# jasonppy/VoiceCraft

Hardware: NVIDIA H100
Metric: codec tokens/s (830M TTS decode) (higher is better)
Workload: dtype bf16

## Files before the change

voicecraft_b200/csrc/lm_engine.cu:

```cuda
#include "../../include/vcb200.h"
#include "lm_kernels.cuh"

#include <algorithm>
#include <array>
#include <cstdarg>
#include <cstdio>
#include <cstdlib>
#include <cstring>
#include <map>
#include <utility>

namespace vcb {

static thread_local char g_err[1024] = "";
void set_error(const char* fmt, ...) {
    va_list ap;
    va_start(ap, fmt);
    vsnprintf(g_err, sizeof(g_err), fmt, ap);
    va_end(ap);
}
const char* get_error() { return g_err; }

__global__ void f32_to_bf16_kernel(const float* __restrict__ in, __nv_bfloat16* __restrict__ out, size_t n) {
    for (size_t i = blockIdx.x * static_cast<size_t>(blockDim.x) + threadIdx.x; i < n;
// ... 106 lines not shown
    DevBuf<__nv_bfloat16> mact_d, mact_d2, mact_f, mact_h;
    DevBuf<int> mega_att_cnt;
    int64_t n_launches = 0;
    struct ProfRec { int cls; Event a, b; };
    std::vector<ProfRec> prof;
    std::vector<Event> ev_pool;
    Event get_event() {
        Event ev;
        if (ev_pool.empty()) {
            ev.create();
        } else {
            ev = std::move(ev_pool.back());
            ev_pool.pop_back();
        }
        return ev;
    }

    ~vcb_engine() {
        cudaSetDevice(cfg.device);
        cudaDeviceSynchronize();
    }
};

enum { PC_GEMM = 0, PC_ATTN = 1, PC_LN = 2, PC_FINISH = 3, PC_SAMPLER = 4, PC_MISC = 5, PC_MEGA = 6, PC_N = 7 };

struct ProfScope {
    vcb_engine* e; cudaStream_t st; int idx = -1;
    ProfScope(vcb_engine* e_, int cls, cudaStream_t st_) : e(e_), st(st_) {
        if (!e->opt_profile) return;
        vcb_engine::ProfRec r{cls, e->get_event(), e->get_event()};
        cudaEventRecord(r.a, st);
        e->prof.push_back(std::move(r));
        idx = static_cast<int>(e->prof.size()) - 1;
    }
    ~ProfScope() { if (idx >= 0) cudaEventRecord(e->prof[idx].b, st); }
};

namespace {

int bpad_for(int rows) { return rows <= 16 ? 16 : rows <= 32 ? 32 : rows <= 64 ? 64 : 128; }
int bpad_idx(int bpad) { return bpad == 16 ? 0 : bpad == 32 ? 1 : bpad == 64 ? 2 : 3; }

int pack_matrix(const float* src, Matrix* M, int rows, int cols) {
    if (M->w.ensure(packed_weight_elems(rows, cols))) return -1;
    M->rows = rows;
    M->cols = cols;
    return pack_weight(src, M->w, rows, cols, &M->tm);
}

int to_bf16_matrix(vcb_engine* e, const std::string& key, Matrix* M, int rows, int cols) {
    auto it = e->f32.find(key);
    if (it == e->f32.end()) {
        set_error("missing weight %s", key.c_str());
        return -1;
    }
    const auto& sh = e->shapes[key];
    if (sh.size() != 2 || sh[0] != rows || sh[1] != cols) {
        set_error("weight %s has wrong shape", key.c_str());
        return -1;
    }
    return pack_matrix(it->second, M, rows, cols);
}

int need(vcb_engine* e, const std::string& key, float** out, size_t numel) {
    auto it = e->f32.find(key);
    if (it == e->f32.end()) {
        set_error("missing weight %s", key.c_str());
        return -1;
    }
    size_t n = 1;
    for (auto s : e->shapes[key]) n *= static_cast<size_t>(s);
    if (n != numel) {
        set_error("weight %s: expected %zu elements, got %zu", key.c_str(), numel, n);
        return -1;
    }
    *out = it->second;
    return 0;
}

int upload_ints(vcb_engine* e, const int* src, size_t n, int* dst, cudaStream_t st) {
    if (n > e->h_stage_ints) {
        set_error("staging overflow");
        return -1;
    }
    VCB_CUDA_OK(cudaEventSynchronize(e->stage_ev));
    memcpy(e->h_stage, src, n * sizeof(int));
    VCB_CUDA_OK(cudaMemcpyAsync(dst, e->h_stage, n * sizeof(int), cudaMemcpyHostToDevice, st));
    VCB_CUDA_OK(cudaEventRecord(e->stage_ev, st));
    return 0;
}

#define LAUNCH_COUNT(e) ((e)->n_launches++)

template <typename... KArgs, typename... Args>
cudaError_t launch_k(vcb_engine* e, void (*kern)(KArgs...), dim3 grid, dim3 block, size_t smem, cudaStream_t st,
                     Args&&... args) {
    return launch_k_pdl(e->opt_pdl, kern, grid, block, smem, st, std::forward<Args>(args)...);
}

int decode_splits(int s, int Nout, int bpad, int maxctas) {
    if (bpad >= 64 && s > 1) s /= 2;
    if (maxctas > 0) {
        const int tiles = (Nout + 127) / 128;
        while (s > 1 && tiles * s > maxctas) s /= 2;
    }
    while (s > 1 && bpad % s) s /= 2;
    return s;
}

int run_gemm(vcb_engine* e, const Matrix& W, const CUtensorMap* tmB, const __nv_bfloat16* X, int ldx, int bpad,
             int nvalid, int b_col_off, int kdim, const GemmEpilogue& ep, cudaStream_t st, const Matrix* next = nullptr) {
    GemmCall g;
    if (next && e->opt_prefetch) {
        g.pf_ptr = next->w;
        g.pf_bytes = packed_weight_elems(next->rows, next->cols) * 2;
        if (e->opt_prefetch == 2) g.pf_bytes |= (1ull << 63);
    }
    g.tmA = &W.tm;
    g.tmB = tmB;
    g.W = W.w;
    g.X = X;
    g.ep = ep;
    g.Nout = W.rows;
    g.Kdim = kdim;
    g.ldx = ldx;
    g.bpad = bpad;
    int splits = gemm_pick_splits(W.rows, kdim, e->num_sms);
    for (const auto& o : e->opt_splits)
        if (o[0] == W.rows && o[1] == kdim) splits = o[2];
    g.splits = decode_splits(splits, W.rows, bpad, e->opt_gemm_maxctas);
    g.stages = e->opt_gemm_stages;
    g.b_col_off = b_col_off;
    g.nvalid = nvalid;
    g.pdl = e->opt_pdl;
    g.simt = e->opt_simt;
    LAUNCH_COUNT(e);
    ProfScope ps(e, PC_GEMM, st);
    return gemm_launch(g, st);
}

struct AttnLaunch {
    const float* q = nullptr;
    const void *kpool = nullptr, *vpool = nullptr;
    const int *page_table = nullptr, *row_slot = nullptr, *row_pos = nullptr;
    const int* row_pages = nullptr;
    int max_pages = 0, rows = 0, H = 0, hd = 0, kv_fp32 = 0, max_ctx = 0;
    __nv_bfloat16* act = nullptr;
    int ld_act = 0, bpad = 0;
    float* ws = nullptr;
    int* cnt = nullptr;
    int maxch = 1, chunk_pages = 16, num_sms = 132, balance = 1, pdl = 0;
    const int *grp_first = nullptr, *grp_shared = nullptr;
    int n_groups = 0;
};

template <typename KVT, int HD, int GMAX>
int launch_attn_hd(const AttnLaunch& a, cudaStream_t st) {
    const float scale = 1.0f / sqrtf(static_cast<float>(HD));
    using L = AttSmem<KVT, HD>;
    static bool set = false;
    if (!set) {
        VCB_CUDA_OK(cudaFuncSetAttribute(attn_rows_kernel<KVT, HD, GMAX>, cudaFuncAttributeMaxDynamicSharedMemorySize, L::TOTAL));
        set = true;
    }
    const int npages = (a.max_ctx + KV_PAGE - 1) / KV_PAGE;
    const int nch = std::min(a.maxch, std::max(1, (npages + a.chunk_pages - 1) / a.chunk_pages));
    const int n_rh = (GMAX == 1 ? a.rows : a.n_groups) * a.H;
    const int per_sm = std::max(1, std::min(4, (227 * 1024) / (L::TOTAL + 1024)));
    int grid = std::min(n_rh * nch, a.num_sms * per_sm);
    if (a.balance) {
        const int items = n_rh * nch, passes = (items + grid - 1) / grid;
        grid = (items + passes - 1) / passes;
    }
    VCB_CUDA_OK(launch_k_pdl(a.pdl, attn_rows_kernel<KVT, HD, GMAX>, dim3(grid), dim3(ATT_THREADS + 32), L::TOTAL, st, a.q,
                             static_cast<const KVT*>(a.kpool), static_cast<const KVT*>(a.vpool), a.page_table, a.max_pages,
                             a.row_slot, a.row_pos, a.H, a.act, a.ld_act, a.bpad, scale, a.ws, a.cnt, a.maxch, a.chunk_pages,
                             n_rh, nch, a.row_pages, a.grp_first, a.grp_shared));
    return 0;
}

template <typename KVT, int HD>
int launch_attn_kv(const AttnLaunch& a, cudaStream_t st) {
    return a.n_groups > 0 ? launch_attn_hd<KVT, HD, ATT_GMAX>(a, st) : launch_attn_hd<KVT, HD, 1>(a, st);
}

int launch_attn_rows(const AttnLaunch& a, cudaStream_t st) {
    if (a.hd != 64 && a.hd != 128) {
        set_error("attention: head dim %d (64 or 128 supported)", a.hd);
        return -1;
    }
    if (a.kv_fp32)
        return a.hd == 128 ? launch_attn_kv<float, 128>(a, st) : launch_attn_kv<float, 64>(a, st);
    return a.hd == 128 ? launch_attn_kv<__nv_bfloat16, 128>(a, st) : launch_attn_kv<__nv_bfloat16, 64>(a, st);
}

struct Plane {
    __nv_bfloat16* act = nullptr;
    const CUtensorMap* tm = nullptr;
};

struct Pass {
    int rows = 0;
    int bpad = 0;
    int max_ctx = 1;
    bool fold = false;
    bool wide = false;
    const int *slot = nullptr, *pos = nullptr, *last = nullptr, *page = nullptr;
    const int* pages = nullptr;
    const int* forced = nullptr;
    const int *grp_first = nullptr, *grp_shared = nullptr;
    int n_groups = 0;
    float* x = nullptr;
    const int* x_index = nullptr;
    float* q = nullptr;
    Plane act_d, act_d2, act_f, act_h;
    float* att_ws = nullptr;
    int* att_cnt = nullptr;
};

Pass narrow_pass(vcb_engine* e, int rows, bool fold) {
    Pass p;
    p.rows = rows;
    p.bpad = bpad_for(rows);
    const int bi = bpad_idx(p.bpad);
    p.fold = fold;
    p.x = e->x_rows;
    p.q = e->qbuf;
    p.act_d = {e->act_d, &e->tm_act_d[bi]};
    p.act_d2 = {e->act_d2, &e->tm_act_d2[bi]};
    p.act_f = {e->act_f, &e->tm_act_f[bi]};
    p.act_h = {e->act_h, &e->tm_act_h[bi]};
    p.att_ws = e->att_ws;
    p.att_cnt = e->att_cnt;
    return p;
}

Pass step_pass(vcb_engine* e, int n, bool fold) {
    Pass p = narrow_pass(e, n, fold);
    p.slot = e->row_slot;
    p.pos = e->row_pos;
    p.last = e->row_last;
    p.page = e->row_page;
    p.pages = e->row_pages;
    p.forced = e->row_forced;
    p.n_groups = e->n_row_groups;
    p.grp_first = e->d_slots + n;
    p.grp_shared = p.grp_first + p.n_groups + 1;
    return p;
}

Pass wide_pass(vcb_engine* e, int rows) {
    Pass p;
    p.rows = rows;
    p.bpad = e->wide_rows;
    p.wide = true;
    p.x = e->wx;
    p.q = e->wq;
    p.act_d = {e->wact_d, &e->tm_wact_d};
    p.act_f = {e->wact_f, &e->tm_wact_f};
    p.att_ws = e->w_att_ws;
    p.att_cnt = e->w_att_cnt;
    return p;
}

void fold_epilogue(GemmEpilogue& ep, const float* cvec, const float* bprime, const float* stats, int tiles, int d) {
    ep.ln_fold = 1;
    ep.cvec = cvec;
    ep.bias = bprime;
    ep.stats = stats;
    ep.stats_tiles = tiles;
    ep.inv_d = 1.0f / static_cast<float>(d);
    ep.ln_d = d;
    ep.ln_eps = 1e-5f;
}

void emit_epilogue(GemmEpilogue& ep, const float* gamma_next, __nv_bfloat16* dst, int d, int bpad, float* stats) {
    ep.emit = 1;
    ep.next_gamma = gamma_next;
    ep.next_act = dst;
    ep.next_ld = d;
    ep.next_bpad = bpad;
    ep.stats_out = stats;
}

struct LayerEpilogues {
    GemmEpilogue qkv, out, ff1, ff2;
};

LayerEpilogues layer_epilogues(const vcb_engine* e, int l, const Pass& p) {
    const ModelDims& m = e->m;
    const Layer& Ly = e->layers[l];
    const int dtiles = (m.d + 127) / 128;
    LayerEpilogues r;
    GemmEpilogue& q = r.qkv;
    q.mode = EPI_QKV;
    q.bias = Ly.b_qkv;
    q.qbuf = p.q;
    q.kpool = Ly.kpool;
    q.vpool = Ly.vpool;
    q.page_table = e->page_table;
    q.row_slot = p.slot;
    q.row_pos = p.pos;
    q.row_page = p.page;
    q.kv_fp32 = e->kv_fp32;
    q.max_pages = e->max_pages_per_slot;
    q.page_size = KV_PAGE;
    q.d = m.d;
    q.H = m.H;
    q.hd = m.hd;
    r.out.mode = EPI_RESID;
    r.out.bias = Ly.b_out;
    r.out.x = p.x;
    r.out.ld_out = m.d;
    r.ff1.mode = EPI_ACT;
    r.ff1.bias = Ly.b_ff1;
    r.ff1.act = p.act_f.act;
    r.ff1.ld_out = m.F;
    r.ff1.act_kind = 1;
    r.ff1.bpad_out = p.bpad;
    r.ff2.mode = EPI_RESID;
    r.ff2.bias = Ly.b_ff2;
    r.ff2.x = p.x;
    r.ff2.ld_out = m.d;
    if (p.fold) {
        fold_epilogue(r.qkv, Ly.c_qkv, Ly.bp_qkv, e->ln_stats, l == 0 ? 1 : dtiles, m.d);
        emit_epilogue(r.out, Ly.ln2_g, p.act_d2.act, m.d, p.bpad, e->ln_stats);
        fold_epilogue(r.ff1, Ly.c_ff1, Ly.bp_ff1, e->ln_stats, dtiles, m.d);
        emit_epilogue(r.ff2, l + 1 < m.L ? e->layers[l + 1].ln1_g : e->lnf_g, p.act_d.act, m.d, p.bpad, e->ln_stats);
    }
    return r;
}

GemmEpilogue heads_epilogue(const vcb_engine* e, const Pass& p) {
    const ModelDims& m = e->m;
    GemmEpilogue ep;
    ep.mode = EPI_ACT;
    ep.bias = e->b_h1;
    ep.act = p.act_h.act;
    ep.ld_out = m.K * m.Hh;
    ep.act_kind = 2;
    ep.bpad_out = p.bpad;
    if (p.fold) fold_epilogue(ep, e->c_h1, e->bp_h1, e->ln_stats, (m.d + 127) / 128, m.d);
    return ep;
}

int pass_gemm(vcb_engine* e, const Pass& p, const Matrix& W, const Plane& in, const GemmEpilogue& ep, cudaStream_t st,
              const Matrix* next) {
    if (!p.wide) return run_gemm(e, W, in.tm, in.act, W.cols, p.bpad, p.rows, 0, W.cols, ep, st, next);
    RowsGemmCall g;
    g.tmX = in.tm;
    g.tmW = &W.tm;
    g.ep = ep;
    g.rows = p.rows;
    g.rcap = p.bpad;
    g.Nout = W.rows;
    g.Kdim = W.cols;
    g.pdl = e->opt_pdl;
    LAUNCH_COUNT(e);
    ProfScope ps(e, PC_GEMM, st);
    return gemm_rows_launch(g, st);
}

int launch_attn(vcb_engine* e, const Pass& p, const Layer& Ly, cudaStream_t st) {
    const ModelDims& m = e->m;
    AttnLaunch a;
    a.q = p.q;
    a.kpool = Ly.kpool;
    a.vpool = Ly.vpool;
    a.page_table = e->page_table;
    a.row_slot = p.slot;
    a.row_pos = p.pos;
    a.row_pages = p.pages;
    a.max_pages = e->max_pages_per_slot;
    a.rows = p.rows;
    a.H = m.H;
    a.hd = m.hd;
    a.kv_fp32 = e->kv_fp32;
    a.max_ctx = p.max_ctx;
    a.act = p.act_d.act;
    a.ld_act = m.d;
    a.bpad = p.bpad;
    a.ws = p.att_ws;
    a.cnt = p.att_cnt;
    a.maxch = e->att_maxch;
    a.chunk_pages = e->att_chunk_pages;
    a.num_sms = e->num_sms;
    a.balance = e->opt_att_balance;
    a.pdl = e->opt_pdl;
    a.grp_first = p.grp_first;
    a.grp_shared = p.grp_shared;
    a.n_groups = p.n_groups;
    ProfScope ps(e, PC_ATTN, st);
    if (launch_attn_rows(a, st)) return -1;
    LAUNCH_COUNT(e);
    return 0;
}

int launch_ln(vcb_engine* e, const Pass& p, const float* g, const float* b, cudaStream_t st) {
    const int d = e->m.d;
    ProfScope ps(e, PC_LN, st);
    auto* kern = d <= 2048 ? ln_rows_kernel<8> : ln_rows_kernel<16>;
    VCB_CUDA_OK(launch_k(e, kern, dim3(p.rows), dim3(256), 0, st, p.x, p.x_index, g, b, p.act_d.act, d, p.bpad, d, 1e-5f));
    LAUNCH_COUNT(e);
    return 0;
}

int forward_layers(vcb_engine* e, const Pass& p, cudaStream_t st) {
    const ModelDims& m = e->m;
    for (int l = 0; l < m.L; ++l) {
        const Layer& Ly = e->layers[l];
        const LayerEpilogues ep = layer_epilogues(e, l, p);
        if (!p.fold && launch_ln(e, p, Ly.ln1_g, Ly.ln1_b, st)) return -1;
        if (pass_gemm(e, p, Ly.qkv, p.act_d, ep.qkv, st, &Ly.out) || launch_attn(e, p, Ly, st) ||
            pass_gemm(e, p, Ly.out, p.act_d, ep.out, st, &Ly.ff1))
            return -1;
        if (!p.fold && launch_ln(e, p, Ly.ln2_g, Ly.ln2_b, st)) return -1;
        if (pass_gemm(e, p, Ly.ff1, p.fold ? p.act_d2 : p.act_d, ep.ff1, st, &Ly.ff2) ||
            pass_gemm(e, p, Ly.ff2, p.act_f, ep.ff2, st, l + 1 < m.L ? &e->layers[l + 1].qkv : &e->h1))
            return -1;
    }
    return 0;
}

bool wide_usable(const vcb_engine* e) {
    const ModelDims& m = e->m;
    return e->opt_prefill_wide && !e->opt_simt && m.hd % 32 == 0 && gemm_rows_supported(3 * m.d, m.d, m.hd) &&
           gemm_rows_supported(m.F, m.d, 0) && gemm_rows_supported(m.d, m.F, 0) && (m.hd == 128 || m.hd == 64);
}

int wide_alloc(vcb_engine* e) {
    const ModelDims& m = e->m;
    const size_t W = static_cast<size_t>(e->wide_rows);
    auto grab = [](auto& buf, size_t n) {
        if (!buf.ensure(n, true)) return false;
        set_error("wide prefill: out of device memory (%zu elements)", n);
        return true;
    };
    if (grab(e->wx, W * m.d) || grab(e->wq, W * m.d) || grab(e->wact_d, 2 * W * m.d) || grab(e->wact_f, 2 * W * m.F) ||
        grab(e->w_att_ws, W * m.H * e->att_maxch * (m.hd + 2)) || grab(e->w_att_cnt, W * m.H))
        return -1;
    if (make_tmap_bf16_2d(&e->tm_wact_d, e->wact_d, 2 * W, m.d, m.d, 128) ||
        make_tmap_bf16_2d(&e->tm_wact_f, e->wact_f, 2 * W, m.F, m.F, 128))
        return -1;
    return 0;
}

int launch_sampler(vcb_engine* e, const Pass& p, const float* noise, const vcb_sampling* sp, cudaStream_t st);

int mega_build(vcb_engine* e, int bpad) {
    const ModelDims& m = e->m;
    const int which = bpad == 32;
    Pass p = step_pass(e, bpad, true);
    p.act_d = {e->mact_d, nullptr};
    p.act_d2 = {e->mact_d2, nullptr};
    p.act_f = {e->mact_f, nullptr};
    p.act_h = {e->mact_h, nullptr};
    std::vector<MegaPhase> ph;
    auto gemm = [&](const CUtensorMap* tm, const void* const* wp, int Nout, int Kdim, int b_map) {
        MegaPhase P;
        P.type = MEGA_GEMM;
        P.tmA = tm;
        P.wptr = wp;
        P.Nout = Nout;
        P.tiles_per_group = (Nout + 127) / 128;
        P.kb = Kdim / 64;
        P.b_map = b_map;
        P.done_target = P.tiles_per_group;
        return P;
    };
    for (int l = 0; l < m.L; ++l) {
        const Layer& Ly = e->layers[l];
        const CUtensorMap* tm = e->d_wmaps + 4 * l;
        const void* const* wp = e->d_wptrs + 4 * l;
        const LayerEpilogues ep = layer_epilogues(e, l, p);
        MegaPhase q = gemm(tm + 0, wp + 0, 3 * m.d, m.d, 0);
        q.ep = ep.qkv;
        q.ep.knew = e->knew;
        q.ep.vnew = e->vnew;
        ph.push_back(q);
        MegaPhase a;
        a.type = MEGA_ATTN;
        a.kpool = Ly.kpool;
        a.vpool = Ly.vpool;
        a.done_target = e->mega_grid;
        ph.push_back(a);
        MegaPhase o = gemm(tm + 1, wp + 1, m.d, m.d, 0);
        o.ep = ep.out;
        ph.push_back(o);
        MegaPhase f1 = gemm(tm + 2, wp + 2, m.F, m.d, 1);
        f1.ep = ep.ff1;
        ph.push_back(f1);
        MegaPhase f2 = gemm(tm + 3, wp + 3, m.d, m.F, 2);
        f2.ep = ep.ff2;
        ph.push_back(f2);
    }
    MegaPhase h1 = gemm(e->d_wmaps + 4 * m.L, e->d_wptrs + 4 * m.L, m.K * m.Hh, m.d, 0);
    h1.ep = heads_epilogue(e, p);
    ph.push_back(h1);
    MegaPhase h2 = gemm(e->d_h2_maps, e->d_wptrs + 4 * m.L + 1, m.V, m.Hh, 3);
    h2.groups = m.K;
    h2.b_grp_stride = m.Hh;
    h2.col_grp_stride = m.Vpad;
    h2.grp_bias = e->d_bias2;
    h2.done_target = m.K * h2.tiles_per_group;
    h2.ep.mode = EPI_LOGITS; h2.ep.out = e->logits; h2.ep.ld_out = m.K * m.Vpad; h2.ep.col_off = 0;
    ph.push_back(h2);
    for (auto& P : ph) {
        if (P.type != MEGA_GEMM) continue;
        const long long T = static_cast<long long>(P.groups) * P.tiles_per_group * P.kb;
        const int Ge = static_cast<int>(std::min<long long>(e->mega_grid, T));
        int segs = 0;
        for (int c = 0; c < Ge; ++c) {
            const long long b0 = T * c / Ge, b1 = T * (c + 1) / Ge;
            segs += static_cast<int>((b1 - 1) / P.kb - b0 / P.kb + 1);
        }
        P.done_target = segs;
    }
    for (size_t i = 1; i < ph.size(); ++i) ph[i].dep_target = ph[i - 1].done_target;
    e->mega_nph = static_cast<int>(ph.size());
    if (e->d_mega_ph[which].ensure(ph.size())) return -1;
    VCB_CUDA_OK(cudaMemcpy(e->d_mega_ph[which], ph.data(), ph.size() * sizeof(MegaPhase), cudaMemcpyHostToDevice));
    return 0;
}

int mega_setup(vcb_engine* e) {
    const ModelDims& m = e->m;
    e->mega_grid = 0;
    if (!e->opt_mega || !e->opt_fold || e->opt_simt || m.hd != 128 || m.d % 128 || m.F % 128 || (m.K * m.Hh) % 128 || m.Hh % 64) return 0;
    int grid = std::min(mega_max_grid(32, e->kv_fp32), mega_max_grid(16, e->kv_fp32));
    if (getenv("VCB_MEGA_GRID")) grid = std::min(grid, atoi(getenv("VCB_MEGA_GRID")));
    if (grid < 1) return 0;
    const int shapes[6][2] = {{3 * m.d / 128, m.d / 64}, {m.d / 128, m.d / 64}, {m.F / 128, m.d / 64}, {m.d / 128, m.F / 64},
                              {m.K * m.Hh / 128, m.d / 64}, {m.K * ((m.V + 127) / 128), m.Hh / 64}};
    int max_tiles = 0;
    for (auto& sh : shapes) {
        const long long T = static_cast<long long>(sh[0]) * sh[1];
        const long long per = (T + grid - 1) / grid;
        if ((per + sh[1] - 1) / sh[1] + 1 > MEGA_MAXSEG) return 0;
        if (T * (grid + 1) >= (1ll << 31)) return 0;
        max_tiles = std::max(max_tiles, sh[0]);
    }
    e->mega_cnt_stride = max_tiles;
    const int nph = 5 * m.L + 2;
    const int R = vcb_engine::MAX_ROWS;
// ... 1263 lines not shown
```

voicecraft_b200/csrc/lm_kernels.cuh:

```cuda
#pragma once
#include "vcb_internal.h"

namespace vcb {

static constexpr int KV_PAGE = 64;
static constexpr int ATT_CWARPS = 8;
static constexpr int ATT_THREADS = ATT_CWARPS * 32;
static constexpr int ATT_STAGES = 3;
static constexpr int ATT_CHUNK_PAGES = 16;
static constexpr int ATT_GMAX = 8;

__device__ __forceinline__ float block_sum_256(float v, float* red ) {
    v = warp_sum(v);
    const int w = threadIdx.x >> 5, l = threadIdx.x & 31;
    __syncthreads();
    if (l == 0) red[w] = v;
    __syncthreads();
    float t = 0.f;
#pragma unroll
    for (int i = 0; i < 8; ++i) t += red[i];
    return t;
}

struct EmbedSeq {
// ... 134 lines not shown
    static constexpr int PAGE_BYTES = KV_PAGE * HD * sizeof(KVT);
    static constexpr int OFF_V = ATT_STAGES * PAGE_BYTES;
    static constexpr int OFF_SC = 2 * ATT_STAGES * PAGE_BYTES;
    static constexpr int OFF_PW = OFF_SC + 2 * KV_PAGE * 4;
    static constexpr int OFF_RED = OFF_PW + ATT_CWARPS * KV_PAGE * 4;
    static constexpr int OFF_BAR = OFF_RED + ATT_CWARPS * HD * 4;
    static constexpr int TOTAL = OFF_BAR + 2 * ATT_STAGES * 8 + 128;
};

template <typename KVT, int N>
__device__ __forceinline__ void load_kv_vec(const KVT* p, float (&out)[N]) {
    if constexpr (sizeof(KVT) == 2) {
        if constexpr (N == 8) {
            const uint4 u = *reinterpret_cast<const uint4*>(p);
            const uint32_t w[4] = {u.x, u.y, u.z, u.w};
#pragma unroll
            for (int i = 0; i < 4; ++i) {
                out[2 * i] = __uint_as_float(w[i] << 16);
                out[2 * i + 1] = __uint_as_float(w[i] & 0xffff0000u);
            }
        } else if constexpr (N == 4) {
            const uint2 u = *reinterpret_cast<const uint2*>(p);
            out[0] = __uint_as_float(u.x << 16);
            out[1] = __uint_as_float(u.x & 0xffff0000u);
            out[2] = __uint_as_float(u.y << 16);
            out[3] = __uint_as_float(u.y & 0xffff0000u);
        } else {
            const uint32_t u = *reinterpret_cast<const uint32_t*>(p);
            out[0] = __uint_as_float(u << 16);
            out[1] = __uint_as_float(u & 0xffff0000u);
        }
    } else {
#pragma unroll
        for (int i = 0; i < N; i += 2) {
            const float2 f = *reinterpret_cast<const float2*>(p + i);
            out[i] = f.x;
            out[i + 1] = f.y;
        }
    }
}

__device__ __forceinline__ void named_bar_sync(int id, int nthreads) {
    asm volatile("bar.sync %0, %1;" ::"r"(id), "r"(nthreads) : "memory");
}

template <typename KVT, int HD>
__device__ __forceinline__ void att_page(const KVT* K, const KVT* V, float* sc, float* pw, const float (&q)[8], int p,
                                         int pos, float scale, float& m_run, float& l_run, float (&acc)[HD / 32]) {
    constexpr int LPT = HD / 8;
    constexpr int TPW = 32 / LPT;
    constexpr int DPT = HD / 32;
    const int warp = threadIdx.x >> 5, lane = threadIdx.x & 31;
    const int sub = lane % LPT;
    constexpr int KPW = KV_PAGE / ATT_CWARPS;
#pragma unroll
    for (int itq = 0; itq < KPW / TPW; ++itq) {
        const int t = warp * KPW + itq * TPW + lane / LPT;
        float kv[8];
        load_kv_vec<KVT, 8>(K + t * HD + sub * 8, kv);
        float dsum = 0.f;
#pragma unroll
        for (int i = 0; i < 8; ++i) dsum = fmaf(q[i], kv[i], dsum);
#pragma unroll
        for (int o = LPT / 2; o > 0; o >>= 1) dsum += __shfl_xor_sync(0xffffffffu, dsum, o);
        if (sub == 0) sc[t] = (p * KV_PAGE + t <= pos) ? dsum * scale : -INFINITY;
    }
    named_bar_sync(1, ATT_THREADS);
    const float s0 = sc[lane], s1 = sc[lane + 32];
    const float m_new = fmaxf(m_run, warp_max(fmaxf(s0, s1)));
    const float corr = expf(m_run - m_new);
    const float e0 = expf(s0 - m_new), e1 = expf(s1 - m_new);
    float* mypw = pw + warp * KV_PAGE;
    mypw[lane] = e0;
    mypw[lane + 32] = e1;
    l_run = l_run * corr + warp_sum(e0 + e1);
    m_run = m_new;
    __syncwarp();
#pragma unroll
    for (int i = 0; i < DPT; ++i) acc[i] *= corr;
#pragma unroll
    for (int tt = 0; tt < KPW; ++tt) {
        const int t = warp * KPW + tt;
        const float pt_ = mypw[t];
        float vv[DPT];
        load_kv_vec<KVT, DPT>(V + t * HD + lane * DPT, vv);
#pragma unroll
        for (int i = 0; i < DPT; ++i) acc[i] = fmaf(pt_, vv[i], acc[i]);
    }
    __syncwarp();
}

template <int HD>
__device__ __forceinline__ void att_finish(const float (&acc)[HD / 32], float m_run, float l_run, int r, int h, int rh,
                                           int chunk, int nch, float* red, __nv_bfloat16* __restrict__ act, int ld_act,
                                           int bpad, float* __restrict__ ws, int* __restrict__ cnt, int maxch, int& s_last) {
    constexpr int DPT = HD / 32;
    const int warp = threadIdx.x >> 5, lane = threadIdx.x & 31;
#pragma unroll
    for (int i = 0; i < DPT; ++i) red[warp * HD + lane * DPT + i] = acc[i];
    named_bar_sync(1, ATT_THREADS);
    const size_t ocol = static_cast<size_t>(h) * HD;
    if (nch == 1) {
        for (int dd = threadIdx.x; dd < HD; dd += ATT_THREADS) {
            float osum = 0.f;
#pragma unroll
            for (int w = 0; w < ATT_CWARPS; ++w) osum += red[w * HD + dd];
            const float o = osum / l_run;
            __nv_bfloat16 hi, lo;
            split_bf16(o, hi, lo);
            act[static_cast<size_t>(r) * ld_act + ocol + dd] = hi;
            act[static_cast<size_t>(r + bpad) * ld_act + ocol + dd] = lo;
        }
        named_bar_sync(1, ATT_THREADS);
        return;
    }
    float* myws = ws + (static_cast<size_t>(rh) * maxch + chunk) * (HD + 2);
    for (int dd = threadIdx.x; dd < HD; dd += ATT_THREADS) {
        float osum = 0.f;
#pragma unroll
        for (int w = 0; w < ATT_CWARPS; ++w) osum += red[w * HD + dd];
        myws[dd] = osum;
    }
    if (threadIdx.x == 0) {
        myws[HD] = m_run;
        myws[HD + 1] = l_run;
    }
    __threadfence();
    named_bar_sync(1, ATT_THREADS);
    if (threadIdx.x == 0) s_last = (atomicAdd(&cnt[rh], 1) == nch - 1);
    named_bar_sync(1, ATT_THREADS);
    if (s_last) {
        __threadfence();
        const volatile float* base = ws + static_cast<size_t>(rh) * maxch * (HD + 2);
        float M = -INFINITY;
        for (int c = 0; c < nch; ++c) M = fmaxf(M, base[c * (HD + 2) + HD]);
        for (int dd = threadIdx.x; dd < HD; dd += ATT_THREADS) {
            float Lsum = 0.f, O = 0.f;
            for (int c = 0; c < nch; ++c) {
                const float w = expf(base[c * (HD + 2) + HD] - M);
                Lsum += base[c * (HD + 2) + HD + 1] * w;
                O += base[c * (HD + 2) + dd] * w;
            }
            const float o = O / Lsum;
            __nv_bfloat16 hi, lo;
            split_bf16(o, hi, lo);
            act[static_cast<size_t>(r) * ld_act + ocol + dd] = hi;
            act[static_cast<size_t>(r + bpad) * ld_act + ocol + dd] = lo;
        }
        if (threadIdx.x == 0) cnt[rh] = 0;
    }
    named_bar_sync(1, ATT_THREADS);
}

template <typename KVT, int HD, int GMAX>
__global__ void __launch_bounds__(ATT_THREADS + 32)
attn_rows_kernel(const float* __restrict__ qbuf, const KVT* __restrict__ kpool, const KVT* __restrict__ vpool,
                 const int* __restrict__ page_table, int max_pages, const int* __restrict__ row_slot,
                 const int* __restrict__ row_pos, int H, __nv_bfloat16* __restrict__ act, int ld_act, int bpad,
                 float scale, float* __restrict__ ws, int* __restrict__ cnt, int maxch, int chunk_pages, int n_rh,
                 int n_chunks, const int* __restrict__ row_pages, const int* __restrict__ grp_first,
                 const int* __restrict__ grp_shared) {
    using L = AttSmem<KVT, HD>;
    constexpr int LPT = HD / 8;
    constexpr int TPW = 32 / LPT;
    constexpr int DPT = HD / 32;
    extern __shared__ __align__(128) uint8_t att_smem[];
    KVT* sK = reinterpret_cast<KVT*>(att_smem);
    KVT* sV = reinterpret_cast<KVT*>(att_smem + L::OFF_V);
    float* sc_all = reinterpret_cast<float*>(att_smem + L::OFF_SC);
    float* pw = reinterpret_cast<float*>(att_smem + L::OFF_PW);
    float* red = reinterpret_cast<float*>(att_smem + L::OFF_RED);
    uint64_t* full = reinterpret_cast<uint64_t*>(att_smem + L::OFF_BAR);
    uint64_t* empty = full + ATT_STAGES;
    __shared__ int s_last;

    const int warp = threadIdx.x >> 5, lane = threadIdx.x & 31;
    pdl_launch_dependents();
    if (threadIdx.x == 0) {
        for (int s = 0; s < ATT_STAGES; ++s) {
            mbar_init(&full[s], 1);
            mbar_init(&empty[s], ATT_CWARPS);
        }
        mbar_fence_init();
        tl_mark(0x300);
        tl_mark_all(0x300);
    }
    __syncthreads();
    pdl_wait();
    if (threadIdx.x == 0) { tl_mark(0x310); tl_mark_all(0x310); }
    const int n_items = n_rh * n_chunks;

    if constexpr (GMAX == 1) {
        if (warp == ATT_CWARPS) {
            if (lane == 0) {
                const uint64_t pol = l2_policy_evict_first();
                int it = 0;
                for (int item = blockIdx.x; item < n_items; item += gridDim.x) {
                    const int chunk = item / n_rh, rh = item - chunk * n_rh;
                    const int r = rh / H, h = rh - r * H;
                    const int pos = row_pos[r];
                    if (pos < 0) continue;
                    const int npages = pos / KV_PAGE + 1;
                    const int p0 = chunk * chunk_pages;
                    if (p0 >= npages) continue;
                    const int p1 = min(npages, p0 + chunk_pages);
                    const int* pt = row_pages ? row_pages + r * max_pages : page_table + row_slot[r] * max_pages;
                    for (int p = p0; p < p1; ++p, ++it) {
                        const int s = it % ATT_STAGES;
                        if (it >= ATT_STAGES) mbar_wait(&empty[s], ((it / ATT_STAGES) - 1) & 1);
                        const size_t off = (static_cast<size_t>(pt[p]) * H + h) * KV_PAGE * HD;
                        mbar_arrive_expect_tx(&full[s], 2 * L::PAGE_BYTES);
                        tma_bulk_g2s_hint(sK + s * KV_PAGE * HD, kpool + off, L::PAGE_BYTES, &full[s], pol);
                        tma_bulk_g2s_hint(sV + s * KV_PAGE * HD, vpool + off, L::PAGE_BYTES, &full[s], pol);
                    }
                }
            }
            return;
        }

        const int sub = lane % LPT;
        int it = 0;
        for (int item = blockIdx.x; item < n_items; item += gridDim.x) {
            const int chunk = item / n_rh, rh = item - chunk * n_rh;
            const int r = rh / H, h = rh - r * H;
            const int pos = row_pos[r];
            if (pos < 0) continue;
            const int npages = pos / KV_PAGE + 1;
            const int p0 = chunk * chunk_pages;
            if (p0 >= npages) continue;
            const int p1 = min(npages, p0 + chunk_pages);
            const int nch = (npages + chunk_pages - 1) / chunk_pages;
            float q[8];
            {
                const float* qp = qbuf + (static_cast<size_t>(r) * H + h) * HD + sub * 8;
    #pragma unroll
                for (int i = 0; i < 8; ++i) q[i] = qp[i];
            }
            float m_run = -INFINITY, l_run = 0.f;
            float acc[DPT];
    #pragma unroll
            for (int i = 0; i < DPT; ++i) acc[i] = 0.f;

            for (int p = p0; p < p1; ++p, ++it) {
                const int s = it % ATT_STAGES;
                mbar_wait(&full[s], (it / ATT_STAGES) & 1);
                const KVT* K = sK + s * KV_PAGE * HD;
                const KVT* V = sV + s * KV_PAGE * HD;
                float* sc = sc_all + (it & 1) * KV_PAGE;
                constexpr int KPW = KV_PAGE / ATT_CWARPS;
    #pragma unroll
                for (int itq = 0; itq < KPW / TPW; ++itq) {
                    const int t = warp * KPW + itq * TPW + lane / LPT;
                    float kv[8];
                    load_kv_vec<KVT, 8>(K + t * HD + sub * 8, kv);
                    float dsum = 0.f;
    #pragma unroll
                    for (int i = 0; i < 8; ++i) dsum = fmaf(q[i], kv[i], dsum);
    #pragma unroll
                    for (int o = LPT / 2; o > 0; o >>= 1) dsum += __shfl_xor_sync(0xffffffffu, dsum, o);
                    if (sub == 0) sc[t] = (p * KV_PAGE + t <= pos) ? dsum * scale : -INFINITY;
                }
                named_bar_sync(1, ATT_THREADS);
                const float s0 = sc[lane], s1 = sc[lane + 32];
                const float m_new = fmaxf(m_run, warp_max(fmaxf(s0, s1)));
                const float corr = expf(m_run - m_new);
                const float e0 = expf(s0 - m_new), e1 = expf(s1 - m_new);
                float* mypw = pw + warp * KV_PAGE;
                mypw[lane] = e0;
                mypw[lane + 32] = e1;
                l_run = l_run * corr + warp_sum(e0 + e1);
                m_run = m_new;
                __syncwarp();
    #pragma unroll
                for (int i = 0; i < DPT; ++i) acc[i] *= corr;
    #pragma unroll
                for (int tt = 0; tt < KPW; ++tt) {
                    const int t = warp * KPW + tt;
                    const float pt_ = mypw[t];
                    float vv[DPT];
                    load_kv_vec<KVT, DPT>(V + t * HD + lane * DPT, vv);
    #pragma unroll
                    for (int i = 0; i < DPT; ++i) acc[i] = fmaf(pt_, vv[i], acc[i]);
                }
                __syncwarp();
                if (lane == 0) mbar_arrive(&empty[s]);
            }
    #pragma unroll
            for (int i = 0; i < DPT; ++i) red[warp * HD + lane * DPT + i] = acc[i];
            named_bar_sync(1, ATT_THREADS);
            const size_t ocol = static_cast<size_t>(h) * HD;
            if (nch == 1) {
                for (int dd = threadIdx.x; dd < HD; dd += ATT_THREADS) {
                    float osum = 0.f;
    #pragma unroll
                    for (int w = 0; w < ATT_CWARPS; ++w) osum += red[w * HD + dd];
                    const float o = osum / l_run;
                    __nv_bfloat16 hi, lo;
                    split_bf16(o, hi, lo);
                    act[static_cast<size_t>(r) * ld_act + ocol + dd] = hi;
                    act[static_cast<size_t>(r + bpad) * ld_act + ocol + dd] = lo;
                }
                named_bar_sync(1, ATT_THREADS);
                continue;
            }
            float* myws = ws + (static_cast<size_t>(rh) * maxch + chunk) * (HD + 2);
            for (int dd = threadIdx.x; dd < HD; dd += ATT_THREADS) {
                float osum = 0.f;
    #pragma unroll
                for (int w = 0; w < ATT_CWARPS; ++w) osum += red[w * HD + dd];
                myws[dd] = osum;
            }
            if (threadIdx.x == 0) {
                myws[HD] = m_run;
                myws[HD + 1] = l_run;
            }
            __threadfence();
            named_bar_sync(1, ATT_THREADS);
            if (threadIdx.x == 0) s_last = (atomicAdd(&cnt[rh], 1) == nch - 1);
            named_bar_sync(1, ATT_THREADS);
            if (s_last) {
                __threadfence();
                const volatile float* base = ws + static_cast<size_t>(rh) * maxch * (HD + 2);
                float M = -INFINITY;
                for (int c = 0; c < nch; ++c) M = fmaxf(M, base[c * (HD + 2) + HD]);
                for (int dd = threadIdx.x; dd < HD; dd += ATT_THREADS) {
                    float Lsum = 0.f, O = 0.f;
                    for (int c = 0; c < nch; ++c) {
                        const float w = expf(base[c * (HD + 2) + HD] - M);
                        Lsum += base[c * (HD + 2) + HD + 1] * w;
                        O += base[c * (HD + 2) + dd] * w;
                    }
                    const float o = O / Lsum;
                    __nv_bfloat16 hi, lo;
                    split_bf16(o, hi, lo);
                    act[static_cast<size_t>(r) * ld_act + ocol + dd] = hi;
                    act[static_cast<size_t>(r + bpad) * ld_act + ocol + dd] = lo;
                }
                if (threadIdx.x == 0) cnt[rh] = 0;
            }
            named_bar_sync(1, ATT_THREADS);
        }
    } else {
        auto pages_of = [&](int r) { return row_pages ? row_pages + r * max_pages : page_table + row_slot[r] * max_pages; };
        auto group_of = [&](int gh, int& r0, int& size, int& h, unsigned& live, int& pos) {
            const int g = gh / H;
            h = gh - g * H;
            r0 = grp_first[g];
            size = grp_first[g + 1] - r0;
            live = 0;
            pos = -1;
#pragma unroll
            for (int j = 0; j < GMAX; ++j)
                if (j < size && row_pos[r0 + j] >= 0) {
                    live |= 1u << j;
                    pos = row_pos[r0 + j];
                }
        };
        if (warp == ATT_CWARPS) {
            if (lane == 0) {
                const uint64_t pol = l2_policy_evict_first();
                int it = 0;
                for (int item = blockIdx.x; item < n_items; item += gridDim.x) {
                    const int chunk = item / n_rh, gh = item - chunk * n_rh;
                    int r0, size, h, pos;
                    unsigned live;
                    group_of(gh, r0, size, h, live, pos);
                    if (!live) continue;
                    const int npages = pos / KV_PAGE + 1;
                    const int p0 = chunk * chunk_pages;
                    if (p0 >= npages) continue;
                    const int p1 = min(npages, p0 + chunk_pages);
                    const int S = grp_shared[gh / H];
                    const int lead = r0 + __ffs(live) - 1;
                    for (int p = p0; p < p1; ++p) {
                        for (int j = 0; j < size; ++j) {
                            if (!(live >> j & 1) || (p < S && r0 + j != lead)) continue;
                            const int s = it % ATT_STAGES;
                            if (it >= ATT_STAGES) mbar_wait(&empty[s], ((it / ATT_STAGES) - 1) & 1);
                            const size_t off = (static_cast<size_t>(pages_of(r0 + j)[p]) * H + h) * KV_PAGE * HD;
                            mbar_arrive_expect_tx(&full[s], 2 * L::PAGE_BYTES);
                            tma_bulk_g2s_hint(sK + s * KV_PAGE * HD, kpool + off, L::PAGE_BYTES, &full[s], pol);
                            tma_bulk_g2s_hint(sV + s * KV_PAGE * HD, vpool + off, L::PAGE_BYTES, &full[s], pol);
                            ++it;
                        }
                    }
                }
            }
            return;
        }

        const int sub = lane % LPT;
        int it = 0, k = 0;
        for (int item = blockIdx.x; item < n_items; item += gridDim.x) {
            const int chunk = item / n_rh, gh = item - chunk * n_rh;
            int r0, size, h, pos;
            unsigned live;
            group_of(gh, r0, size, h, live, pos);
            if (!live) continue;
            const int npages = pos / KV_PAGE + 1;
            const int p0 = chunk * chunk_pages;
            if (p0 >= npages) continue;
            const int p1 = min(npages, p0 + chunk_pages);
            const int nch = (npages + chunk_pages - 1) / chunk_pages;
            const int S = grp_shared[gh / H];
            float q[GMAX][8], m_run[GMAX], l_run[GMAX], acc[GMAX][DPT];
#pragma unroll
            for (int j = 0; j < GMAX; ++j) {
                if (live >> j & 1) {
                    const float* qp = qbuf + (static_cast<size_t>(r0 + j) * H + h) * HD + sub * 8;
#pragma unroll
                    for (int i = 0; i < 8; ++i) q[j][i] = qp[i];
                }
                m_run[j] = -INFINITY;
                l_run[j] = 0.f;
#pragma unroll
                for (int i = 0; i < DPT; ++i) acc[j][i] = 0.f;
            }
            for (int p = p0; p < p1; ++p) {
                const bool shared = p < S;
#pragma unroll
                for (int j = 0; j < GMAX; ++j) {
                    if (!(live >> j & 1)) continue;
                    const int s = it % ATT_STAGES;
                    const bool first = !shared || (live & ((1u << j) - 1)) == 0;
                    const bool last = !shared || (live >> (j + 1)) == 0;
                    if (first) mbar_wait(&full[s], (it / ATT_STAGES) & 1);
                    att_page<KVT, HD>(sK + s * KV_PAGE * HD, sV + s * KV_PAGE * HD, sc_all + (k & 1) * KV_PAGE, pw, q[j], p,
                                      pos, scale, m_run[j], l_run[j], acc[j]);
                    ++k;
                    if (last) {
                        if (lane == 0) mbar_arrive(&empty[s]);
                        ++it;
                    }
                }
            }
#pragma unroll
            for (int j = 0; j < GMAX; ++j)
                if (live >> j & 1)
                    att_finish<HD>(acc[j], m_run[j], l_run[j], r0 + j, h, (r0 + j) * H + h, chunk, nch, red, act, ld_act,
                                   bpad, ws, cnt, maxch, s_last);
        }
    }
    if (threadIdx.x == 0) { tl_mark(0x330); tl_mark_all(0x330); }
}

__global__ void __launch_bounds__(256)
step_prep_kernel(const int* __restrict__ slots, int n, SlotState* __restrict__ st, const GroupState* __restrict__ gr,
                 int* __restrict__ row_slot, int* __restrict__ row_pos, int* __restrict__ row_last,
                 const float* __restrict__ x_slot, float* __restrict__ x_rows, int d,
                 const float* __restrict__ gamma0, __nv_bfloat16* __restrict__ act, int bpad, float* __restrict__ stats,
                 const int* __restrict__ page_table, int max_pages, int* __restrict__ row_page,
                 int* __restrict__ row_pages, int* __restrict__ row_forced, unsigned int* __restrict__ phase_flags,
                 int n_phase_flags, unsigned int* __restrict__ tile_counters, int n_tile_counters,
                 __nv_bfloat16* __restrict__ act_tiled) {
    __shared__ float red[8];
    pdl_launch_dependents();
    pdl_wait();
    const int r = blockIdx.x;
    if (r == 0)
        for (int i = threadIdx.x; i < n_phase_flags; i += blockDim.x) phase_flags[i] = 0u;
    for (int i = r * blockDim.x + threadIdx.x; i < n_tile_counters; i += gridDim.x * blockDim.x) tile_counters[i] = 0u;
    const int slot = slots[r];
    __shared__ int s_pos;
    if (threadIdx.x == 0) {
        SlotState& S = st[slot];
        const bool on = S.active && !gr[S.group].done;
        s_pos = on ? S.seq_len : -1;
        row_slot[r] = slot;
        row_pos[r] = s_pos;
        row_last[r] = on ? slot : -1;
        row_page[r] = on ? page_table[slot * max_pages + s_pos / KV_PAGE] : 0;
        row_forced[r] = S.forced;
        if (on) {
            S.seq_len += 1;
            S.y_len += 1;
        }
    }
    for (int j = threadIdx.x; j < max_pages; j += blockDim.x)
        row_pages[static_cast<size_t>(r) * max_pages + j] = page_table[slot * max_pages + j];
    __syncthreads();
    if (s_pos < 0) return;
    float s1 = 0.f, s2 = 0.f;
    for (int c = threadIdx.x; c < d; c += blockDim.x) {
        const float v = x_slot[static_cast<size_t>(slot) * d + c];
        x_rows[static_cast<size_t>(r) * d + c] = v;
        if (gamma0) {
            __nv_bfloat16 hi, lo;
            split_bf16(gamma0[c] * v, hi, lo);
            act[static_cast<size_t>(r) * d + c] = hi;
            act[static_cast<size_t>(r + bpad) * d + c] = lo;
            if (act_tiled) {
                const int kk = c & 63, rows2 = 2 * bpad;
                const size_t t0 = static_cast<size_t>(c >> 6) * rows2;
                act_tiled[(t0 + r) * 64 + ((((kk >> 3) ^ (r & 7)) << 3) | (kk & 7))] = hi;
// ... 567 lines not shown
```

Before: 64640.

## Prefetch first KV pages in attention kernel before PDL dependency wait

Before the programmatic-dependent-launch wait, the producer thread reads the slot's sequence length from slot state and issues TMA loads for the first few KV pages of the block's first work item. This overlaps KV fetch latency with the tail of the preceding kernel. Consumers drain any prefetched stages that go unused so the mbarrier phases stay consistent. The risk is reading slot state or page tables before the prior kernel has finished writing them, and the bookkeeping adds complexity to the pipeline.

After: 67240 (median of 6 runs). 1.04x the previous value.

```diff
diff --git a/voicecraft_b200/csrc/lm_engine.cu b/voicecraft_b200/csrc/lm_engine.cu
--- a/voicecraft_b200/csrc/lm_engine.cu
+++ b/voicecraft_b200/csrc/lm_engine.cu
@@ -282,6 +282,8 @@
     int maxch = 1, chunk_pages = 16, num_sms = 132, balance = 1, pdl = 0;
     const int *grp_first = nullptr, *grp_shared = nullptr;
     int n_groups = 0;
+    const int* pre_slot = nullptr;
+    const SlotState* pre_state = nullptr;
 };
 
 template <typename KVT, int HD, int GMAX>
@@ -305,7 +307,7 @@
     VCB_CUDA_OK(launch_k_pdl(a.pdl, attn_rows_kernel<KVT, HD, GMAX>, dim3(grid), dim3(ATT_THREADS + 32), L::TOTAL, st, a.q,
                              static_cast<const KVT*>(a.kpool), static_cast<const KVT*>(a.vpool), a.page_table, a.max_pages,
                              a.row_slot, a.row_pos, a.H, a.act, a.ld_act, a.bpad, scale, a.ws, a.cnt, a.maxch, a.chunk_pages,
-                             n_rh, nch, a.row_pages, a.grp_first, a.grp_shared));
+                             n_rh, nch, a.row_pages, a.grp_first, a.grp_shared, a.pre_slot, a.pre_state));
     return 0;
 }
 
@@ -340,6 +342,8 @@
     const int* forced = nullptr;
     const int *grp_first = nullptr, *grp_shared = nullptr;
     int n_groups = 0;
+    const int* pre_slot = nullptr;
+    const SlotState* pre_state = nullptr;
     float* x = nullptr;
     const int* x_index = nullptr;
     float* q = nullptr;
@@ -376,6 +380,8 @@
     p.n_groups = e->n_row_groups;
     p.grp_first = e->d_slots + n;
     p.grp_shared = p.grp_first + p.n_groups + 1;
+    p.pre_slot = e->d_slots;
+    p.pre_state = e->st;
     return p;
 }
 
@@ -520,6 +526,8 @@
     a.grp_first = p.grp_first;
     a.grp_shared = p.grp_shared;
     a.n_groups = p.n_groups;
+    a.pre_slot = p.pre_slot;
+    a.pre_state = p.pre_state;
     ProfScope ps(e, PC_ATTN, st);
     if (launch_attn_rows(a, st)) return -1;
     LAUNCH_COUNT(e);
diff --git a/voicecraft_b200/csrc/lm_kernels.cuh b/voicecraft_b200/csrc/lm_kernels.cuh
--- a/voicecraft_b200/csrc/lm_kernels.cuh
+++ b/voicecraft_b200/csrc/lm_kernels.cuh
@@ -310,6 +310,31 @@
     named_bar_sync(1, ATT_THREADS);
 }
 
+template <typename KVT, int HD>
+__device__ __forceinline__ int att_pages_before_wait(const KVT* kpool, const KVT* vpool, const int* page_table, int max_pages,
+                                                     const int* slots, const SlotState* state, int H, int chunk_pages,
+                                                     int n_rh, int n_items, KVT* sK, KVT* sV, uint64_t* full) {
+    using L = AttSmem<KVT, HD>;
+    const int item = blockIdx.x;
+    if (item >= n_items) return 0;
+    const int chunk = item / n_rh, rh = item - chunk * n_rh;
+    const int r = rh / H, h = rh - r * H;
+    const int slot = slots[r];
+    const int len = *reinterpret_cast<const volatile int*>(&state[slot].seq_len);
+    const int p0 = chunk * chunk_pages;
+    const int p1 = min(min((len - 1) / KV_PAGE, p0 + chunk_pages), p0 + ATT_STAGES);
+    const int* pt = page_table + static_cast<size_t>(slot) * max_pages;
+    const uint64_t pol = l2_policy_evict_first();
+    int n = 0;
+    for (int p = p0; p < p1; ++p, ++n) {
+        const size_t off = (static_cast<size_t>(pt[p]) * H + h) * KV_PAGE * HD;
+        mbar_arrive_expect_tx(&full[n], 2 * L::PAGE_BYTES);
+        tma_bulk_g2s_hint(sK + n * KV_PAGE * HD, kpool + off, L::PAGE_BYTES, &full[n], pol);
+        tma_bulk_g2s_hint(sV + n * KV_PAGE * HD, vpool + off, L::PAGE_BYTES, &full[n], pol);
+    }
+    return n;
+}
+
 template <typename KVT, int HD, int GMAX>
 __global__ void __launch_bounds__(ATT_THREADS + 32)
 attn_rows_kernel(const float* __restrict__ qbuf, const KVT* __restrict__ kpool, const KVT* __restrict__ vpool,
@@ -317,7 +342,7 @@
                  const int* __restrict__ row_pos, int H, __nv_bfloat16* __restrict__ act, int ld_act, int bpad,
                  float scale, float* __restrict__ ws, int* __restrict__ cnt, int maxch, int chunk_pages, int n_rh,
                  int n_chunks, const int* __restrict__ row_pages, const int* __restrict__ grp_first,
-                 const int* __restrict__ grp_shared) {
+                 const int* __restrict__ grp_shared, const int* __restrict__ pre_slot, const SlotState* pre_state) {
     using L = AttSmem<KVT, HD>;
     constexpr int LPT = HD / 8;
     constexpr int TPW = 32 / LPT;
@@ -330,29 +355,34 @@
     float* red = reinterpret_cast<float*>(att_smem + L::OFF_RED);
     uint64_t* full = reinterpret_cast<uint64_t*>(att_smem + L::OFF_BAR);
     uint64_t* empty = full + ATT_STAGES;
-    __shared__ int s_last;
+    __shared__ int s_last, s_pre;
 
     const int warp = threadIdx.x >> 5, lane = threadIdx.x & 31;
+    const int n_items = n_rh * n_chunks;
     pdl_launch_dependents();
-    if (threadIdx.x == 0) {
+    if (threadIdx.x == 0) { tl_mark(0x300); tl_mark_all(0x300); }
+    if (threadIdx.x == ATT_THREADS) {
         for (int s = 0; s < ATT_STAGES; ++s) {
             mbar_init(&full[s], 1);
             mbar_init(&empty[s], ATT_CWARPS);
         }
         mbar_fence_init();
-        tl_mark(0x300);
-        tl_mark_all(0x300);
+        int pre = 0;
+        if constexpr (GMAX == 1)
+            if (pre_slot) pre = att_pages_before_wait<KVT, HD>(kpool, vpool, page_table, max_pages, pre_slot, pre_state, H,
+                                                              chunk_pages, n_rh, n_items, sK, sV, full);
+        s_pre = pre;
     }
     __syncthreads();
     pdl_wait();
     if (threadIdx.x == 0) { tl_mark(0x310); tl_mark_all(0x310); }
-    const int n_items = n_rh * n_chunks;
+    const int n_pre = s_pre;
 
     if constexpr (GMAX == 1) {
         if (warp == ATT_CWARPS) {
             if (lane == 0) {
                 const uint64_t pol = l2_policy_evict_first();
-                int it = 0;
+                int it = n_pre;
                 for (int item = blockIdx.x; item < n_items; item += gridDim.x) {
                     const int chunk = item / n_rh, rh = item - chunk * n_rh;
                     const int r = rh / H, h = rh - r * H;
@@ -363,7 +393,7 @@
                     if (p0 >= npages) continue;
                     const int p1 = min(npages, p0 + chunk_pages);
                     const int* pt = row_pages ? row_pages + r * max_pages : page_table + row_slot[r] * max_pages;
-                    for (int p = p0; p < p1; ++p, ++it) {
+                    for (int p = item == blockIdx.x ? p0 + n_pre : p0; p < p1; ++p, ++it) {
                         const int s = it % ATT_STAGES;
                         if (it >= ATT_STAGES) mbar_wait(&empty[s], ((it / ATT_STAGES) - 1) & 1);
                         const size_t off = (static_cast<size_t>(pt[p]) * H + h) * KV_PAGE * HD;
@@ -377,16 +407,26 @@
         }
 
         const int sub = lane % LPT;
-        int it = 0;
+        int it = 0, owed = 0;
+        auto drain = [&]() {
+            for (; owed > 0; --owed, ++it) {
+                const int s = it % ATT_STAGES;
+                mbar_wait(&full[s], (it / ATT_STAGES) & 1);
+                __syncwarp();
+                if (lane == 0) mbar_arrive(&empty[s]);
+            }
+        };
         for (int item = blockIdx.x; item < n_items; item += gridDim.x) {
+            drain();
             const int chunk = item / n_rh, rh = item - chunk * n_rh;
             const int r = rh / H, h = rh - r * H;
             const int pos = row_pos[r];
-            if (pos < 0) continue;
             const int npages = pos / KV_PAGE + 1;
             const int p0 = chunk * chunk_pages;
+            const int p1 = min(npages, p0 + chunk_pages);
+            if (item == blockIdx.x) owed = max(0, n_pre - (pos >= 0 ? max(0, p1 - p0) : 0));
+            if (pos < 0) continue;
             if (p0 >= npages) continue;
-            const int p1 = min(npages, p0 + chunk_pages);
             const int nch = (npages + chunk_pages - 1) / chunk_pages;
             float q[8];
             {
@@ -498,6 +538,7 @@
             }
             named_bar_sync(1, ATT_THREADS);
         }
+        drain();
     } else {
         auto pages_of = [&](int r) { return row_pages ? row_pages + r * max_pages : page_table + row_slot[r] * max_pages; };
         auto group_of = [&](int gh, int& r0, int& size, int& h, unsigned& live, int& pos) {
```
